# dohyeon-Lee/IsaacgymEnv

Hardware: AMD Instinct MI355X
Metric: env-steps/sec AnymalTerrain 4096 envs/GPU (higher is better)
Workload: dtype f32; 1 GPU; AnymalTerrain VecTask.step, terrainType plane (AnymalTerrain.yaml default), 5 physics substeps/step, obs noise on; num_envs_per_gpu=4096, global_num_envs=4096, parallelism=dp1, solver=TGS (physx.solver_type 1, cfg/config.yaml:31)

## Files before the change

isaacgymenv_amd/csrc/gs_capi.hip:

```cpp
#include <cmath>
#include <cstdio>
#include <cstring>
#include <algorithm>
#include <chrono>
#include <string>
#include <vector>

#include "gs_internal.h"
#include "../../include/gymsim.h"

namespace {
thread_local std::string g_err;

int fail(const char* fmt, const char* arg = nullptr) {
  char buf[512];
  std::snprintf(buf, sizeof(buf), fmt, arg ? arg : "");
  g_err = buf;
  return -1;
}
int hip_fail(hipError_t e, const char* where) {
  char buf[512];
  std::snprintf(buf, sizeof(buf), "%s: %s", where, hipGetErrorString(e));
  g_err = buf;
  return -1;
// ... 99 lines not shown
    if (hipError_t e = hipSetDevice(device); e != hipSuccess) {
      hip_fail(e, "gs_sim_create hipSetDevice");
      return nullptr;
    }
    s = new gs_sim();
    s->device = device;
  }
  s->params = *p;
  const int sub = p->substeps > 0 ? p->substeps : 1;
  s->dp.h = (float)(p->dt / sub);
  s->dp.substeps = sub;
  for (int k = 0; k < 3; ++k) s->dp.g[k] = (float)p->gravity[k];
  s->dp.pos_iters = p->num_position_iterations;
  s->dp.vel_iters = p->num_velocity_iterations;
  s->dp.contact_offset = (float)p->contact_offset;
  s->dp.rest_offset = (float)p->rest_offset;
  s->dp.max_depen_vel = (float)p->max_depenetration_velocity;
  s->dp.tgs = p->solver_type == 1 && p->num_position_iterations > 0 ? 1 : 0;
  s->dp.collect = p->contact_collection != 0;
  s->dp.limit_margin = (float)(p->joint_limit_margin > 0 ? p->joint_limit_margin : 0.0);
  s->dp.any_limits = 0;
  s->dp.has_ground = 0;
  s->dp.ground_mu = 1.f;
  return s;
}

void gs_sim_destroy(gs_sim* s) {
  if (!s) return;
  if (s->host) {
    host_pool_destroy(s->pool);
    delete s;
    return;
  }
  (void)hipSetDevice(s->device);
  if (s->d_model) (void)hipFree(s->d_model);
  if (s->d_links) (void)hipFree(s->d_links);
  if (s->d_tverts) (void)hipFree(s->d_tverts);
  if (s->d_tcells) (void)hipFree(s->d_tcells);
  if (s->d_tblk) (void)hipFree(s->d_tblk);
  if (s->d_tsq4) (void)hipFree(s->d_tsq4);
  if (s->d_trec) (void)hipFree(s->d_trec);
  if (s->d_rows) (void)hipFree(s->d_rows);
  if (s->d_gen) (void)hipFree(s->d_gen);
  if (s->ev0) (void)hipEventDestroy(s->ev0);
  if (s->ev1) (void)hipEventDestroy(s->ev1);
  delete s;
// ... 857 lines not shown
```

isaacgymenv_amd/csrc/gs_internal.h:

```cpp
#pragma once
#include <hip/hip_runtime.h>

#include "gs_terrain.h"
#include "../../include/gymtask.h"

#define GS_MAXB 32
#define GS_MAXD 32
#define GS_MAXC 192
#define GS_MAXL 40
#define GS_MAXS 8
#define GS_MAXSH 32
#define GS_MAXHV 2048
#define GS_MAXP 512
#define GS_MAXPV 512
#define GS_MAXPOOL 8
#define GS_WAVE 64
#ifndef GS_MIN_RESPONSE
#define GS_MIN_RESPONSE 1e-3f
#endif

struct DevModel {
  float jR[GS_MAXB][9];
  float jt[GS_MAXB][3];
  float jaxis[GS_MAXB][3];
// ... 29 lines not shown
struct DevParams {
  float h;
  int substeps;
  float g[3];
  int pos_iters, vel_iters;
  int tgs;
  float contact_offset, rest_offset, max_depen_vel;
  float ground_mu;
  int has_ground;
  int collect;
  float limit_margin;
  int any_limits;
  int has_terrain;
  TerrainDev terr;
  int any_drive;
  int self_collide;
  const float* ptgt;
  const float* vtgt;
  const float* dof_env;
  int dof_env_n;
  const struct GenTopo* gen;
  const struct DevLinks* gen_links;
  int gen_nd, gen_nr;
};
#define GS_DOFP_FIELDS 6

struct SimBuffers {
  float* state;
  const float* mu;
  float* cf;
  int N;
  float* sens;
  float* rows;
};

struct GenTopo {
  int nc;
  int cbody[GS_MAXC], cshape[GS_MAXC], clink[GS_MAXC];
};

struct PdDev {
  const float* actions;
  const float* dof_state_in;
  const float* default_pos;
  float kp, kd, scale, tlim;
  int decimation, extra;
// ... 103 lines not shown
```

isaacgymenv_amd/csrc/gs_team.hip:

```cpp
#include <type_traits>

#include "gs_internal.h"
#include "gs_topologies.h"
#include "gs_math.h"
#include "gs_pairs.h"
#include "gt_anymal_tail.h"

#ifdef GS_PHASE_PROFILE
__device__ unsigned long long gs_phase_cycles[64];
#define GS_PROF_DECL long long gs_t_ = clock64(); long long gs_acc_[16] = {0};
#define GS_PROF(i) { const long long t_ = clock64(); gs_acc_[i] += t_ - gs_t_; gs_t_ = t_; }
#define GS_PROF_COUNT(i, n) { gs_acc_[i] += (n); }
#define GS_PROF_PARAM , long long &gs_t_, long long *gs_acc_
#define GS_PROF_ARGS , gs_t_, gs_acc_
#define GS_PROF_FLUSH                                                   \
  if ((threadIdx.x & 63) == 0) {                                        \
    long long tot_ = 0;                                                 \
    for (int i_ = 0; i_ < 16; ++i_) {                                   \
      atomicAdd(&gs_phase_cycles[i_], (unsigned long long)gs_acc_[i_]); \
      if (i_ < 8 || i_ == 11) tot_ += gs_acc_[i_];                      \
    }                                                                   \
    atomicAdd(&gs_phase_cycles[16 + (int)min(tot_ / 25000, 15ll)], 1ull); \
    if (tot_ > 250000) {                                                \
      for (int i_ = 0; i_ < 16; ++i_) atomicAdd(&gs_phase_cycles[32 + i_], (unsigned long long)gs_acc_[i_]); \
// ... 67 lines not shown
    case 2: return qperm_i<0xAA>(x);
    default: return qperm_i<0xFF>(x);
  }
}

template <class T>
struct CM {
  static constexpr int CL = T::T_CL, CC = T::T_CC;
  static constexpr int BODY = 25;
  static constexpr int CAND = BODY * CL;
  static constexpr int DOF = CAND + 4 * CC;
  static constexpr int SHP = DOF + 3 * CL;
  static constexpr int NP = SHP + (T::NPK > 0 ? 8 * T::T_SPC : 0);
  static constexpr int LANES = T::T_LANES;
};

#ifndef GS_TEAM_BLOCK
#define GS_TEAM_BLOCK 64
#endif
constexpr int kTeamBlock = GS_TEAM_BLOCK;
static_assert(kTeamBlock % 4 == 0 && kTeamBlock <= GS_WAVE, "a workgroup holds whole teams within one wave");

constexpr int RW = kTeamBlock + 1;

template <class T>
struct RowSlots {
  static constexpr int CL = T::T_CL;
  static constexpr int ZROW = 16;
  static constexpr int RZROW = 16;
  static constexpr int CSLOT = 15;
  __device__ static constexpr int zslot(int comp) { return comp < 6 ? 4 * (comp >> 1) + (comp & 1) : 4 * (comp - 6) + 2; }
  __device__ static constexpr int zs(int rr, int s) { return rr < 2 ? 2 * s + rr : 2 * ZROW + s; }
  static constexpr int C_DI = 3 * ZROW, C_G = C_DI + 3, C_TP = C_G + 3, C_TV = C_TP + 1,
                       C_MU = C_TV + 1, C_ACT = C_MU + 1, C_SEP = C_ACT + 1, PER_CONTACT = C_SEP + 1;
  static constexpr int R_DI = 3 * RZROW, R_G = R_DI + 3, R_TP = R_G + 3, R_TV = R_TP + 1,
                       R_MU = R_TV + 1, R_SEP = R_MU + 1, PER_ROOT = R_SEP + 1;
  static constexpr int CHAIN = PER_CONTACT * T::T_CC;
  static constexpr int ROOT = PER_ROOT * (T::T_RC > 0 ? T::T_RC : 1);
  static constexpr int P_Z = kPoolLam + 3, P_DI = P_Z + 15, P_G = P_DI + 3, P_TP = P_G + 3, P_TV = P_TP + 1,
                       P_CA = P_TV + 1, P_CB = P_CA + 1, PER_POOL = P_CB + 1;
  static constexpr int POOL = CHAIN + ROOT;
  static constexpr int TOTAL = POOL + PER_POOL * T::NPK;
  __device__ static constexpr int chain(int j) { return j * PER_CONTACT; }
  __device__ static constexpr int root(int j) { return CHAIN + j * PER_ROOT; }
};

// ... 304 lines not shown
  return -1;
}
template <class T>
__device__ __forceinline__ unsigned long long team_pair_bit(int lc, int ra, int ja, int dl, int jb) {
  unsigned long long bit = 0ull;
#pragma unroll
  for (int c = 0; c < 4; ++c) {
    const int a = ja < 0 ? ra : T::T_RS + c * T::T_SPC + ja;
    const int b = T::T_RS + ((c + dl) & 3) * T::T_SPC + jb;
    const int q = team_pair_index<T>(a, b);
    bit = lc == c ? (q >= 0 ? 1ull << q : 0ull) : bit;
  }
  return bit;
}
__device__ __forceinline__ unsigned long long quad_or64(unsigned long long m) {
  int lo = (int)(unsigned)m, hi = (int)(unsigned)(m >> 32);
  lo |= qperm_i<0xB1>(lo);
  hi |= qperm_i<0xB1>(hi);
  lo |= qperm_i<0x4E>(lo);
  hi |= qperm_i<0x4E>(hi);
  return ((unsigned long long)(unsigned)hi << 32) | (unsigned)lo;
}

template <class T>
__device__ __forceinline__ int team_narrow_replicated(const DevModel* __restrict__ M, const DevParams& P,
                                                   const float* __restrict__ mu_g, int N, int e, int lc,
                                                   const float (&R0)[9], const float (&R)[T::T_CL][9],
                                                   const float (&X)[T::T_CL][3], unsigned long long near,
                                                   float* __restrict__ shw_tab, const float* __restrict__ sct,
                                                   float* __restrict__ pool) {
  constexpr int TPW = kTeamsPerBlock;
  const int team = threadIdx.x >> 2;
  float* tab = shw_tab + team;
  __syncthreads();
#pragma unroll
  for (int j = 0; j < T::T_SPC; ++j) {
    const int sh = T::T_RS + lc * T::T_SPC + j;
    const int k = T::sh_body[T::T_RS + j] - 1;
    const float* ps = sct + ShapeTab<T>::POSE + 15 * sh;
    float Rs[9], t[3], c[3];
    mat3mul(R[k], ps, Rs);
    mat3vec(R[k], ps + 9, t);
    mat3vec(R[k], ps + 12, c);
#pragma unroll
    for (int f = 0; f < 9; ++f) tab[(kShW * sh + f) * TPW] = Rs[f];
#pragma unroll
    for (int f = 0; f < 3; ++f) {
      tab[(kShW * sh + 9 + f) * TPW] = X[k][f] + t[f];
      tab[(kShW * sh + 12 + f) * TPW] = X[k][f] + c[f];
    }
  }
  if (lc == 0) {
#pragma unroll
    for (int sh = 0; sh < T::T_RS; ++sh) {
      const float* ps = sct + ShapeTab<T>::POSE + 15 * sh;
      float Rs[9], t[3], c[3];
      mat3mul(R0, ps, Rs);
      mat3vec(R0, ps + 9, t);
      mat3vec(R0, ps + 12, c);
#pragma unroll
      for (int f = 0; f < 9; ++f) tab[(kShW * sh + f) * TPW] = Rs[f];
#pragma unroll
      for (int f = 0; f < 3; ++f) {
        tab[(kShW * sh + 9 + f) * TPW] = t[f];
        tab[(kShW * sh + 12 + f) * TPW] = c[f];
      }
    }
  }
  __syncthreads();
  const unsigned long long tmask = quad_or64(near);
  int cnt = 0;
  if (tmask) cnt = self_contacts<T, TPW, RW, RowSlots<T>::PER_POOL>(M, P, mu_g, N, e, tab, pool, ShapeConstsTab{sct},
                                                                    tmask);
  return cnt;
}

template <class T>
__device__ __forceinline__ int team_self_contacts(const DevModel* __restrict__ M, const float* __restrict__ cm,
                                                  const DevParams& P, const float* __restrict__ mu_g, int N, int e,
                                                  int lc, const float (&R0)[9], const float (&R)[T::T_CL][9],
                                                  const float (&X)[T::T_CL][3], float* __restrict__ shw_tab,
                                                  const float* __restrict__ sct, float* __restrict__ pool) {
  constexpr int TPW = kTeamsPerBlock, LN = T::T_LANES, SPC = T::T_SPC, RSH = T::T_RS;
  using C = CM<T>;
  const float off = P.contact_offset * 1.001f + 1e-5f;
  float p0[SPC][3], p1[SPC][3], rad[SPC], hl[SPC];
#pragma unroll
  for (int j = 0; j < SPC; ++j) {
    const int k = T::sh_body[RSH + j] - 1;
    const float* sp = cm + (C::SHP + 8 * j) * LN;
    const float l0[3] = {sp[0], sp[LN], sp[2 * LN]}, l1[3] = {sp[3 * LN], sp[4 * LN], sp[5 * LN]};
    mat3vec(R[k], l0, p0[j]);
    mat3vec(R[k], l1, p1[j]);
#pragma unroll
    for (int f = 0; f < 3; ++f) { p0[j][f] += X[k][f]; p1[j][f] += X[k][f]; }
    rad[j] = sp[6 * LN];
    hl[j] = sp[7 * LN];
  }
  static_assert(T::NPAIR <= 64, "the team's near-pair mask is 64 bits");
  unsigned long long near = 0ull;
  auto test = [&](const float* a0, const float* a1, float ra, float ha, bool sa, int, const float* b0, const float* b1,
                  float rb, float hb, bool sb, int, unsigned long long bit) {
    const float rr = ra + rb + off;
    float dc = 0.f;
#pragma unroll
    for (int k = 0; k < 3; ++k) {
// ... 49 lines not shown
          q0[j][g] = dl == 1 ? qperm<0x39>(p0[j][g]) : qperm<0x4E>(p0[j][g]);
          q1[j][g] = dl == 1 ? qperm<0x39>(p1[j][g]) : qperm<0x4E>(p1[j][g]);
        }
      }
      if (dl == 1 || lcv < 2) {
        const int lo = (lcv + dl) & 3;
#pragma unroll
        for (int j = 0; j < SPC; ++j)
#pragma unroll
          for (int j2 = 0; j2 < SPC; ++j2)
            if (team_pair<T>(RSH + j, RSH + SPC + j2))
              f(p0[j], p1[j], rad[j], hl[j], T::shkind[RSH + j] == 1, RSH + lcv * SPC + j, q0[j2], q1[j2], rad[j2],
                hl[j2], T::shkind[RSH + j2] == 1, RSH + lo * SPC + j2, team_pair_bit<T>(lcv, 0, j, dl, j2));
      }
    }
  };
  visit(lc, test);
  if (__ballot(near != 0ull) == 0ull) return 0;
#ifdef GS_PHASE_PROFILE
  if ((threadIdx.x & 63) == 0) atomicAdd(&gs_phase_cycles[12], 1ull);
  const long long np_t0 = clock64();
#endif
  if constexpr (!team_closed_form<T>()) {
    return team_narrow_replicated<T>(M, P, mu_g, N, e, lc, R0, R, X, near, shw_tab, sct, pool);
  } else {
  constexpr int kLC = team_lc<T>(), kSt = kTeamSt;
  constexpr int kNone = 0x7fffffff;
  const int wl = threadIdx.x & 63;
  const int team = threadIdx.x >> 2;
  float* lslot = shw_tab + wl;
  float* tstg = shw_tab + kLC * kSt * 64 + team;
  static_assert(kLC * kSt * 64 + T::NPK * kSt * TPW <= shw_size<T>(), "contact staging fits the table");
  __syncthreads();
  const float coff = P.contact_offset;
  int cnt = 0;
  int key[kLC];
#pragma unroll
  for (int i = 0; i < kLC; ++i) key[i] = kNone;
  auto narrow = [&](const float* a0_, const float* a1_, float ra_, float, bool sa, int ia, const float* b0_,
                    const float* b1_, float rb_, float, bool sb, int ib, unsigned long long bit) {
    if (!(near & bit)) return;
    const int q = __builtin_ctzll(bit);
    const bool sw = ia > ib;
    float a0[3], a1[3], b0[3], b1[3];
#pragma unroll
    for (int k = 0; k < 3; ++k) {
      a0[k] = sw ? b0_[k] : a0_[k]; a1[k] = sw ? b1_[k] : a1_[k];
      b0[k] = sw ? a0_[k] : b0_[k]; b1[k] = sw ? a1_[k] : b1_[k];
    }
    const float ra = sw ? rb_ : ra_, rb = sw ? ra_ : rb_;
    const int sha = sw ? ib : ia, shb = sw ? ia : ib;
    float pa[2][3], pb[2][3];
    int nct = 1;
    if (!sa && !sb) {
#pragma unroll
      for (int k = 0; k < 3; ++k) { pa[0][k] = a0[k]; pb[0][k] = b0[k]; }
// ... 52 lines not shown
        if (!(l > 1e-9f)) { f[0] = 0.f; f[1] = 0.f; f[2] = 1.f; l = 1.f; }
#pragma unroll
        for (int k = 0; k < 3; ++k) nn[k] = f[k] / l;
        dist = 0.f;
      } else {
        const float idist = __builtin_amdgcn_rsqf(d2);
#pragma unroll
        for (int k = 0; k < 3; ++k) nn[k] *= idist;
      }
      const float sep = dist - ra - rb;
      if (!(sep < coff)) continue;
      const int kn = 2 * q + c;
      int slot = cnt < kLC ? cnt : -1;
      if (cnt >= kLC) {
        int m = 0, km = key[0];
#pragma unroll
        for (int i = 1; i < kLC; ++i) {
          m = key[i] > km ? i : m;
          km = key[i] > km ? key[i] : km;
        }
        slot = kn < km ? m : -1;
      }
      if (slot >= 0) {
        float* o = lslot + kSt * slot * 64;
#pragma unroll
        for (int k = 0; k < 3; ++k) {
          o[k * 64] = 0.5f * ((pa[c][k] - ra * nn[k]) + (pb[c][k] + rb * nn[k]));
          o[(3 + k) * 64] = nn[k];
        }
        o[6 * 64] = sep;
        o[7 * 64] = __int_as_float(sha);
        o[8 * 64] = __int_as_float(shb);
#pragma unroll
        for (int i = 0; i < kLC; ++i) key[i] = i == slot ? kn : key[i];
      }
      ++cnt;
    }
  };
  visit(opaque_index(lc), narrow);
#ifdef GS_PHASE_PROFILE
  if ((threadIdx.x & 63) == 0) atomicAdd(&gs_phase_cycles[14], (unsigned long long)(clock64() - np_t0));
#endif
  int cnt_team = 0;
  {
    int rk[kLC];
#pragma unroll
    for (int i = 0; i < kLC; ++i) rk[i] = 0;
    auto tally = [&](const int (&ks)[kLC]) {
#pragma unroll
      for (int j = 0; j < kLC; ++j)
#pragma unroll
        for (int i = 0; i < kLC; ++i) rk[i] += ks[j] < key[i];
    };
    tally(key);
    {
      int ks[kLC];
#pragma unroll
      for (int j = 0; j < kLC; ++j) ks[j] = qperm_i<0x39>(key[j]);
      tally(ks);
#pragma unroll
      for (int j = 0; j < kLC; ++j) ks[j] = qperm_i<0x4E>(key[j]);
      tally(ks);
#pragma unroll
      for (int j = 0; j < kLC; ++j) ks[j] = qperm_i<0x93>(key[j]);
      tally(ks);
    }
    cnt_team = cnt + qperm_i<0xB1>(cnt);
    cnt_team += qperm_i<0x4E>(cnt_team);
#pragma unroll
    for (int i = 0; i < kLC; ++i) {
      if (i < cnt && rk[i] < T::NPK) {
        const float* src = lslot + kSt * i * 64;
        float* dst = tstg + kSt * rk[i] * TPW;
#pragma unroll
        for (int f = 0; f < kSt; ++f) dst[f * TPW] = src[f * 64];
      }
    }
    __syncthreads();
    cnt_team = cnt_team < T::NPK ? cnt_team : T::NPK;
#pragma unroll
    for (int r = 0; r < T::NPK; ++r) {
      if (r < cnt_team) {
        const float* src = tstg + kSt * r * TPW;
        float* o = pool + RowSlots<T>::PER_POOL * r * RW;
#pragma unroll
        for (int k = 0; k < 3; ++k) {
          o[(kPoolX + k) * RW] = src[k * TPW];
          o[(kPoolN + k) * RW] = src[(3 + k) * TPW];
        }
        o[kPoolSep * RW] = src[6 * TPW];
        const int a = __float_as_int(src[7 * TPW]), b = __float_as_int(src[8 * TPW]);
        const float nn[3] = {src[3 * TPW], src[4 * TPW], src[5 * TPW]};
        float t1[3], t2[3];
        gs_terrain::tangents(nn, t1, t2);
#pragma unroll
        for (int k = 0; k < 3; ++k) {
          o[(kPoolT1 + k) * RW] = t1[k];
          o[(kPoolT2 + k) * RW] = t2[k];
        }
        o[kPoolMu * RW] = 0.5f * (mu_g[a * N + e] + mu_g[b * N + e]);
        const int bla = (int)sct[kShC * a + 3], blb = (int)sct[kShC * b + 3];
// ... 14 lines not shown
      atomicAdd(&gs_phase_cycles[10], (unsigned long long)__popcll(tm));
    }
  }
#endif
  return cnt_team;
  }
}

__device__ __forceinline__ float terrain_candidate(const DevParams& P, const float* p, const float* x, float r,
                                                   float* nrm, float& smu) {
  const float cw[3] = {p[0] + x[0], p[1] + x[1], p[2] + x[2]};
  float dist = P.has_ground ? cw[2] - r : 3.0e38f;
  nrm[0] = 0.f; nrm[1] = 0.f; nrm[2] = 1.f;
  smu = P.ground_mu;
  float st, nt[3];
  if (gs_terrain::sphere_contact(P.terr, cw, r, r + P.contact_offset, st, nt) && st < dist) {
    dist = st;
    nrm[0] = nt[0]; nrm[1] = nt[1]; nrm[2] = nt[2];
    smu = P.terr.mu;
  }
  return dist;
}

template <class T, bool TERR, bool TGS>
__device__ __forceinline__ void substep_team(const DevModel* __restrict__ Min, const float* __restrict__ mdl,
                                             const DevParams& P, TeamState<T>& s, const float* tau,
                                             const float* __restrict__ mu_t, int N, int e, int lc,
                                             float* __restrict__ rows_own, const float* __restrict__ rows_team,
                                             float* __restrict__ cf_soa, bool collect,
                                             float* __restrict__ cf_aos, float* __restrict__ shw_tab,
                                             const float* __restrict__ sct, float* __restrict__ stash GS_PROF_PARAM) {
  constexpr int CL = T::T_CL, CC = T::T_CC, RC = T::T_RC, NCH = T::T_NCH, LN = T::T_LANES;
  static_assert(NCH == LN && LN == 4, "lane teams are DPP quads with one chain per lane");
  using C = CM<T>;
  using RS = RowSlots<T>;
  uintptr_t mp = reinterpret_cast<uintptr_t>(Min);
  asm volatile("" : "+s"(mp));
  const DevModel* __restrict__ M = reinterpret_cast<const DevModel*>(mp);
  const float* cm = mdl + lc;
  const float h = P.h;

  float R0[9];
  {
    const float inv = rsqrtf(s.quat[0] * s.quat[0] + s.quat[1] * s.quat[1] + s.quat[2] * s.quat[2] +
                             s.quat[3] * s.quat[3]);
    const float qn[4] = {s.quat[0] * inv, s.quat[1] * inv, s.quat[2] * inv, s.quat[3] * inv};
    quat_to_mat(qn, R0);
// ... 81 lines not shown
      qr[CC] = M->cradius[lc];
    }
    constexpr int kQItem = 9;
    static_assert(T::NPK > 0 && kShW * T::NS >= kQItem * (CC * LN + RC), "query list fits the pose table");
    float* ql = shw_tab;
    const int wl = threadIdx.x & 63;
    const unsigned long long below = (1ull << wl) - 1ull;
    int slot[NQ];
    int cnt = 0;
#ifdef GS_PHASE_PROFILE
    const long long tq0 = clock64();
#endif
#pragma unroll
    for (int q = 0; q < NQ; ++q) {
      const bool need = qv[q] && gs_terrain::may_contact(P.terr, qc[q], qr[q], qr[q] + P.contact_offset);
      const unsigned long long bal = __ballot(need);
      slot[q] = need ? cnt + __popcll(bal & below) : -1;
      if (need) {
        float* it = ql + slot[q] * kQItem;
        it[0] = qc[q][0]; it[1] = qc[q][1]; it[2] = qc[q][2]; it[3] = qr[q];
      }
      cnt += __popcll(bal);
    }
    __syncthreads();
#ifdef GS_PHASE_PROFILE
    const long long tq1 = clock64();
#endif
    const unsigned long long live = __ballot(true);
    const int nlive = __popcll(live);
    for (int i = __popcll(live & below); i < cnt; i += nlive) {
      float* it = ql + i * kQItem;
      const float cw[3] = {it[0], it[1], it[2]};
      const float r = it[3];
      float st = 0.f, nt[3] = {0.f, 0.f, 1.f};
      const bool found = gs_terrain::sphere_contact_scan(P.terr, cw, r, r + P.contact_offset, st, nt);
      it[4] = found ? 1.f : 0.f;
      it[5] = st;
      it[6] = nt[0]; it[7] = nt[1]; it[8] = nt[2];
    }
    __syncthreads();
#ifdef GS_PHASE_PROFILE
    if ((threadIdx.x & 63) == 0) {
      const long long tq2 = clock64();
      atomicAdd(&gs_phase_cycles[50], (unsigned long long)(tq1 - tq0));
      atomicAdd(&gs_phase_cycles[51], (unsigned long long)(tq2 - tq1));
      atomicAdd(&gs_phase_cycles[52], (unsigned long long)cnt);
    }
#endif
    float rd = 3.0e38f, rn[3] = {0.f, 0.f, 1.f}, rm = P.ground_mu;
#pragma unroll
    for (int q = 0; q < NQ; ++q) {
      float dist = P.has_ground ? qc[q][2] - qr[q] : 3.0e38f;
      float nrm[3] = {0.f, 0.f, 1.f};
      float smu = P.ground_mu;
      if (slot[q] >= 0) {
        const float* it = ql + slot[q] * kQItem;
        if (it[4] != 0.f && it[5] < dist) {
          dist = it[5];
          nrm[0] = it[6]; nrm[1] = it[7]; nrm[2] = it[8];
          smu = P.terr.mu;
        }
      }
      if (q < CC) {
// ... 37 lines not shown
    if (T::jkind[1 + k] == 1) {
      float sn, cs;
      sincosf(qj, &sn, &cs);
      const float Cc = 1.f - cs;
      float Rq[9];
      Rq[0] = cs + ax[0] * ax[0] * Cc;         Rq[1] = ax[0] * ax[1] * Cc - ax[2] * sn; Rq[2] = ax[0] * ax[2] * Cc + ax[1] * sn;
      Rq[3] = ax[1] * ax[0] * Cc + ax[2] * sn; Rq[4] = cs + ax[1] * ax[1] * Cc;         Rq[5] = ax[1] * ax[2] * Cc - ax[0] * sn;
      Rq[6] = ax[2] * ax[0] * Cc - ax[1] * sn; Rq[7] = ax[2] * ax[1] * Cc + ax[0] * sn; Rq[8] = cs + ax[2] * ax[2] * Cc;
      mat3mul(RJ, Rq, R[k]);
      S[k][0] = aw[0]; S[k][1] = aw[1]; S[k][2] = aw[2];
      cross3(X[k], aw, &S[k][3]);
    } else {
#pragma unroll
      for (int f = 0; f < 9; ++f) R[k][f] = RJ[f];
      X[k][0] += aw[0] * qj; X[k][1] += aw[1] * qj; X[k][2] += aw[2] * qj;
      S[k][0] = S[k][1] = S[k][2] = 0.f;
      S[k][3] = aw[0]; S[k][4] = aw[1]; S[k][5] = aw[2];
    }
  }
  GS_PROF(0)
  int npc = 0;
  float* pool = rows_own + RS::POOL * RW;
  if constexpr (T::NPK > 0) {
    if (P.self_collide) npc = team_self_contacts<T>(M, cm, P, mu_t, kTeamsPerBlock, 0, lc, R0, R, X, shw_tab, sct, pool);
  }
  GS_PROF(11)
#pragma unroll
  for (int k = 0; k < CL; ++k) {
    const float* Vp = k == 0 ? nub : V[k - 1];
    const float* Ap = k == 0 ? A0 : A[k - 1];
    const float* bp = cm + (k * C::BODY) * LN;
    const float qd = s.qd[k];
    float c6[6];
#pragma unroll
    for (int f = 0; f < 6; ++f) V[k][f] = Vp[f] + S[k][f] * qd;
    crm(V[k], S[k], c6);
#pragma unroll
    for (int f = 0; f < 6; ++f) A[k][f] = Ap[f] + c6[f] * qd;
    float com[3], Il[6];
#pragma unroll
    for (int f = 0; f < 3; ++f) com[f] = bp[(16 + f) * LN];
#pragma unroll
    for (int f = 0; f < 6; ++f) Il[f] = bp[(19 + f) * LN];
    body_inertia(R[k], X[k], bp[15 * LN], com, Il, Ic[k]);
    {
      float ia[6], iv[6], x6[6];
      spi_mul(Ic[k], A[k], ia);
// ... 469 lines not shown
        c21 += zc3[2][k] * zc3[1][k];
      }
      g10 += quad_sum(c10);
      g20 += quad_sum(c20);
      g21 += quad_sum(c21);
      float di[3];
#pragma unroll
      for (int rr = 0; rr < 3; ++rr) {
        di[rr] = dd[rr] > GS_MIN_RESPONSE ? __builtin_amdgcn_rcpf(dd[rr]) : 0.f;
        o[(RS::P_DI + rr) * RW] = di[rr];
        o[(kPoolLam + rr) * RW] = 0.f;
      }
      o[(RS::P_G + 0) * RW] = g10 * di[1];
      o[(RS::P_G + 1) * RW] = g20 * di[2];
      o[(RS::P_G + 2) * RW] = g21 * di[2];
      const float sc = o[kPoolSep * RW];
      const float tgt = -sc * inv_h;
      o[RS::P_TP * RW] = (sc < 0.f ? fminf(tgt, P.max_depen_vel) : tgt) * di[0];
      o[RS::P_TV * RW] = (sc < 0.f ? 0.f : tgt) * di[0];
      o[RS::P_CA * RW] = (float)ca;
      o[RS::P_CB * RW] = (float)(cb == ca ? -1 : cb);
    }
  }
  __syncthreads();

  GS_PROF(3)
  auto stash_io = [&](bool save) {
    int q = 0;
    auto io = [&](float& v) {
      if (save) stash[q * kTeamBlock] = v; else v = stash[q * kTeamBlock];
      ++q;
    };
#pragma unroll
    for (int k = 0; k < 6; ++k) {
#pragma unroll
      for (int b = 0; b < k; ++b) io(Mbb[k][b]);
      io(sDb[k]);
      io(nufb[k]);
    }
#pragma unroll
    for (int k = 0; k < CL; ++k) {
#pragma unroll
      for (int b = 0; b < 6; ++b) io(Mcb[k][b]);
#pragma unroll
      for (int j = 0; j < k; ++j) io(Mcc[k][j]);
      io(sDc[k]);
      io(nufc[k]);
// ... 194 lines not shown
#pragma unroll
      for (int c = 0; c < NCH; ++c) aC[c] += wC[c];
    }
    if (it == P.pos_iters - 1) {
      if constexpr (tgs) {
        const float inv_n = 1.f / (float)P.pos_iters;
        float mC[NCH];
#pragma unroll
        for (int c = 0; c < NCH; ++c) mC[c] = aC[c] * inv_n;
        gather_w<T>(lc, aA * inv_n, aA2 * inv_n, mC, wbp, wcp);
      } else {
        gather_w<T>(lc, wA, wA2, wC, wbp, wcp);
      }
    }
  }
  float wb[6], wc[CL];
  gather_w<T>(lc, wA, wA2, wC, wb, wc);
  if (P.pos_iters <= 0) {
#pragma unroll
    for (int b = 0; b < 6; ++b) wbp[b] = wb[b];
#pragma unroll
    for (int k = 0; k < CL; ++k) wcp[k] = wc[k];
  }
  __syncthreads();
  stash_io(false);

  GS_PROF(4)
  float nunb[6], nupb[6], nunc[CL], nupc[CL];
#pragma unroll
  for (int k = 0; k < 6; ++k) {
    float v = wb[k] * sDb[k], vp = wbp[k] * sDb[k];
#pragma unroll
    for (int b = 0; b < k; ++b) { v -= Mbb[k][b] * nunb[b]; vp -= Mbb[k][b] * nupb[b]; }
    nunb[k] = v;
    nupb[k] = vp;
  }
#pragma unroll
  for (int k = 0; k < CL; ++k) {
    float v = wc[k] * sDc[k], vp = wcp[k] * sDc[k];
#pragma unroll
    for (int b = 0; b < 6; ++b) { v -= Mcb[k][b] * nunb[b]; vp -= Mcb[k][b] * nupb[b]; }
#pragma unroll
    for (int j = 0; j < k; ++j) { v -= Mcc[k][j] * nunc[j]; vp -= Mcc[k][j] * nupc[j]; }
    nunc[k] = v;
    nupc[k] = vp;
  }
#pragma unroll
// ... 113 lines not shown
        float* o = cf_aos + (size_t)e * T::NB * 3;
        o[0] = f0; o[1] = f1; o[2] = f2;
      }
    }
  }
  GS_PROF(5)
}

template <class T>
__device__ __forceinline__ void team_com_velocity(const DevModel* __restrict__ M, const TeamState<T>& s, float* v) {
  float R[9], c[3], wc[3];
  quat_to_mat(s.quat, R);
  mat3vec(R, M->root_com, c);
  cross3(s.w, c, wc);
  v[0] = s.vo[0] + wc[0]; v[1] = s.vo[1] + wc[1]; v[2] = s.vo[2] + wc[2];
}

__device__ __forceinline__ int xcd_block(int b, int G) {
  constexpr int kXcd = 8;
  const int per = G / kXcd, rem = G % kXcd, x = b % kXcd, q = b / kXcd;
  return x * per + (x < rem ? x : rem) + q;
}

template <class T, bool TERR, bool TGS>
__global__ __launch_bounds__(kTeamBlock, 1) void k_simulate_team(const DevModel* __restrict__ M, DevParams P,
                                                                 SimBuffers B, const float* __restrict__ tau_aos) {
  constexpr int LN = T::T_LANES, CL = T::T_CL, ND = T::ND;
  __shared__ float mdl[CM<T>::NP * LN];
  __shared__ float rows[RowSlots<T>::TOTAL * RW];
  __shared__ float shw_tab[shw_size<T>()];
  __shared__ float sct[ShapeTab<T>::SIZE];
  __shared__ float mu_tab[T::NS * kTeamsPerBlock];
  __shared__ float stash_tab[team_stash_size<T>() * kTeamBlock];
  stage_chain_model<T>(M, mdl);
  stage_shape_consts<T>(M, sct);
  const int lc = threadIdx.x & (LN - 1);
  const int e = (xcd_block(blockIdx.x, gridDim.x) * kTeamBlock + threadIdx.x) / LN;
  for (int sh = lc; sh < T::NS; sh += LN)
    mu_tab[sh * kTeamsPerBlock + (threadIdx.x >> 2)] = e < B.N ? B.mu[(size_t)sh * B.N + e] : 1.f;
  __syncthreads();
  if (e >= B.N) return;
  const float* mu_t = mu_tab + (threadIdx.x >> 2);
  const int N = B.N;
  TeamState<T> s;
  team_load<T>(B.state, N, e, lc, s);
  float tau[CL];
#pragma unroll
  for (int k = 0; k < CL; ++k) tau[k] = tau_aos ? tau_aos[(size_t)e * ND + lc * CL + k] : 0.f;
  float* own = rows + threadIdx.x;
  const float* team = rows + (threadIdx.x & ~(LN - 1));
  GS_PROF_DECL
  for (int sstep = 0; sstep < P.substeps; ++sstep) {
    const bool last = (sstep == P.substeps - 1) && P.collect;
    substep_team<T, TERR, TGS>(M, mdl, P, s, tau, mu_t, N, e, lc, own, team, B.cf, last, nullptr, shw_tab, sct, stash_tab + threadIdx.x GS_PROF_ARGS);
  }
  team_store<T>(B.state, N, opaque_index(e), opaque_index(lc), s);
  GS_PROF_FLUSH
}

template <class T, bool TERR, bool TGS>
__global__ __launch_bounds__(kTeamBlock, 1) void k_pd_step_team(const DevModel* __restrict__ M, DevParams P,
                                                                SimBuffers B, PdDev A) {
  constexpr int LN = T::T_LANES, CL = T::T_CL, ND = T::ND, NB = T::NB;
  __shared__ float mdl[CM<T>::NP * LN];
  __shared__ float rows[RowSlots<T>::TOTAL * RW];
  __shared__ float shw_tab[shw_size<T>()];
  __shared__ float sct[ShapeTab<T>::SIZE];
  __shared__ float mu_tab[T::NS * kTeamsPerBlock];
  __shared__ float stash_tab[team_stash_size<T>() * kTeamBlock];
  stage_chain_model<T>(M, mdl);
  stage_shape_consts<T>(M, sct);
  const int lc = threadIdx.x & (LN - 1);
  const int e = (xcd_block(blockIdx.x, gridDim.x) * kTeamBlock + threadIdx.x) / LN;
  for (int sh = lc; sh < T::NS; sh += LN)
    mu_tab[sh * kTeamsPerBlock + (threadIdx.x >> 2)] = e < B.N ? B.mu[(size_t)sh * B.N + e] : 1.f;
  __syncthreads();
  if (e >= B.N) return;
  const float* mu_t = mu_tab + (threadIdx.x >> 2);
  const int N = B.N;
  TeamState<T> s;
  team_load<T>(B.state, N, e, lc, s);
  float tau[CL];
  float* own = rows + threadIdx.x;
  const float* team = rows + (threadIdx.x & ~(LN - 1));
  const int sub = P.substeps;
  const int n_pd = A.decimation * sub;
  const int total = (A.decimation + A.extra) * sub;
  auto dof0 = [&]() { return (size_t)opaque_index(e) * ND + lc * CL; };
  GS_PROF_DECL
  for (int it = 0; it < total; ++it) {
    if (it < n_pd && (it % sub) == 0) {
      const bool first = it == 0;
      const size_t d0 = dof0();
#pragma unroll
      for (int k = 0; k < CL; ++k) {
        const float qj = first ? A.dof_state_in[(d0 + k) * 2 + 0] : s.q[k];
        const float qdj = first ? A.dof_state_in[(d0 + k) * 2 + 1] : s.qd[k];
        const float aj = A.actions[d0 + k];
        tau[k] = clampf(A.kp * (A.scale * aj + A.default_pos[lc * CL + k] - qj) - A.kd * qdj, -A.tlim, A.tlim);
      }
    }
    const bool last = ((it % sub) == sub - 1) && P.collect;
    GS_PROF(6)
    float* cf_aos = (it == total - 1) ? A.cf_out : nullptr;
    substep_team<T, TERR, TGS>(M, mdl, P, s, tau, mu_t, N, e, lc, own, team, B.cf, last, cf_aos, shw_tab, sct, stash_tab + threadIdx.x GS_PROF_ARGS);
    if (it == n_pd - 1 && A.dof_out) {
      const size_t d0 = dof0();
#pragma unroll
      for (int k = 0; k < CL; ++k) {
        A.dof_out[(d0 + k) * 2 + 0] = s.q[k];
        A.dof_out[(d0 + k) * 2 + 1] = s.qd[k];
      }
    }
  }
  team_store<T>(B.state, N, opaque_index(e), opaque_index(lc), s);
  const size_t d0 = dof0();
#pragma unroll
  for (int k = 0; k < CL; ++k) A.torques_out[d0 + k] = tau[k];
  if (A.actions_copy) {
#pragma unroll
    for (int k = 0; k < CL; ++k) A.actions_copy[d0 + k] = A.actions[d0 + k];
  }
  if (A.root_out && lc == 0) {
    float* o = A.root_out + (size_t)e * 13;
    o[0] = s.p[0]; o[1] = s.p[1]; o[2] = s.p[2];
    o[3] = s.quat[0]; o[4] = s.quat[1]; o[5] = s.quat[2]; o[6] = s.quat[3];
    float v[3];
    team_com_velocity<T>(M, s, v);
    o[7] = v[0]; o[8] = v[1]; o[9] = v[2];
    o[10] = s.w[0]; o[11] = s.w[1]; o[12] = s.w[2];
  }
  if constexpr (!TERR) if (kTeamsPerBlock == 16 && A.tail_on) {
    __syncthreads();
    const bool reset = lc == 0 && (ND == 12 ? gt_tail::post_a_env<true, false, (ND == 12 ? 12 : 0)>(
                                                  A.tail_p, A.tail_b, gt_anymal_hound{}, e)
                                            : gt_tail::post_a_env<true, false>(A.tail_p, A.tail_b, gt_anymal_hound{}, e));
    const unsigned long long m = __ballot(reset);
    unsigned m16 = 0;
#pragma unroll
    for (int i = 0; i < kTeamsPerBlock; ++i) m16 |= (unsigned)((m >> (LN * i)) & 1ull) << i;
    const int e0 = e - (int)(threadIdx.x / LN);
    const unsigned long long live = __ballot(true);
    if ((int)(threadIdx.x & 63) == __ffsll((long long)live) - 1) {
      uint16_t* slices = reinterpret_cast<uint16_t*>(A.tail_b.reset_masks);
      slices[e0 / kTeamsPerBlock] = (uint16_t)m16;
      if (e0 + kTeamsPerBlock >= N)
        for (int q = e0 / kTeamsPerBlock + 1; q % 4 != 0; ++q) slices[q] = 0;
      gt_tail::publish_count(A.tail_b, (unsigned)__popc(m16), gridDim.x);
    }
  }
  GS_PROF(7)
  GS_PROF_FLUSH
}

}

bool team_fused_tail_available() { return kTeamsPerBlock == 16; }

template <class T>
hipError_t launch_sim_team(const DevModel* M, const DevParams& P, const SimBuffers& B, const float* tau,
                           hipStream_t st) {
  if constexpr (T::HAS_TEAM) {
    static_assert(T::NR == T::NB, "the lane team reports contact forces per body (no kept fixed-joint links)");
    const long lanes = (long)B.N * T::T_LANES;
    const int blocks = (int)((lanes + kTeamBlock - 1) / kTeamBlock);
    if (P.has_terrain && P.tgs)
      hipLaunchKernelGGL((k_simulate_team<T, true, true>), dim3(blocks), dim3(kTeamBlock), 0, st, M, P, B, tau);
    else if (P.has_terrain)
      hipLaunchKernelGGL((k_simulate_team<T, true, false>), dim3(blocks), dim3(kTeamBlock), 0, st, M, P, B, tau);
    else if (P.tgs)
      hipLaunchKernelGGL((k_simulate_team<T, false, true>), dim3(blocks), dim3(kTeamBlock), 0, st, M, P, B, tau);
    else
      hipLaunchKernelGGL((k_simulate_team<T, false, false>), dim3(blocks), dim3(kTeamBlock), 0, st, M, P, B, tau);
    return hipGetLastError();
  } else {
    return hipErrorInvalidConfiguration;
  }
}
template <class T>
hipError_t launch_pd_team(const DevModel* M, const DevParams& P, const SimBuffers& B, const PdDev& A, hipStream_t st) {
  if constexpr (T::HAS_TEAM) {
    const long lanes = (long)B.N * T::T_LANES;
    const int blocks = (int)((lanes + kTeamBlock - 1) / kTeamBlock);
    if (P.has_terrain && P.tgs)
      hipLaunchKernelGGL((k_pd_step_team<T, true, true>), dim3(blocks), dim3(kTeamBlock), 0, st, M, P, B, A);
    else if (P.has_terrain)
      hipLaunchKernelGGL((k_pd_step_team<T, true, false>), dim3(blocks), dim3(kTeamBlock), 0, st, M, P, B, A);
    else if (P.tgs)
      hipLaunchKernelGGL((k_pd_step_team<T, false, true>), dim3(blocks), dim3(kTeamBlock), 0, st, M, P, B, A);
    else
      hipLaunchKernelGGL((k_pd_step_team<T, false, false>), dim3(blocks), dim3(kTeamBlock), 0, st, M, P, B, A);
    return hipGetLastError();
  } else {
    return hipErrorInvalidConfiguration;
  }
}

#define GS_TEAM_ENTRY(T, SIG) {SIG, T::HAS_TEAM ? &launch_sim_team<T> : nullptr, T::HAS_TEAM ? &launch_pd_team<T> : nullptr},
TeamEntry g_team_kernels[] = {GS_FOR_EACH_TOPOLOGY(GS_TEAM_ENTRY)};
const int g_num_team_kernels = sizeof(g_team_kernels) / sizeof(g_team_kernels[0]);

extern "C" int gs_debug_phase_cycles(unsigned long long* out, int n, int reset) {
#ifdef GS_PHASE_PROFILE
  if (!out || n <= 0 || n > 64) return -1;
  if (hipDeviceSynchronize() != hipSuccess) return -1;
  if (hipMemcpyFromSymbol(out, HIP_SYMBOL(gs_phase_cycles), sizeof(unsigned long long) * n) != hipSuccess) return -1;
  if (reset) {
    unsigned long long z[64] = {0};
    if (hipMemcpyToSymbol(HIP_SYMBOL(gs_phase_cycles), z, sizeof(z)) != hipSuccess) return -1;
  }
  return 0;
#else
  (void)out; (void)n; (void)reset;
  return -1;
// ... 3 lines not shown
```

Before: 31.53 million env-steps/s.

## Split team workgroups into multiple waves with fewer envs per wave on plane

```diff
diff --git a/isaacgymenv_amd/csrc/gs_capi.hip b/isaacgymenv_amd/csrc/gs_capi.hip
--- a/isaacgymenv_amd/csrc/gs_capi.hip
+++ b/isaacgymenv_amd/csrc/gs_capi.hip
@@ -1,4 +1,5 @@
 #include <cmath>
+#include <cstdlib>
 #include <cstdio>
 #include <cstring>
 #include <algorithm>
@@ -145,6 +146,10 @@
   s->dp.any_limits = 0;
   s->dp.has_ground = 0;
   s->dp.ground_mu = 1.f;
+  if (const char* v = std::getenv("GS_TEAM_ENVS_PER_WAVE")) {
+    const int w = std::atoi(v);
+    s->dp.team_epw = w == 16 || w == 8 || w == 4 ? w : 0;
+  }
   return s;
 }
 
diff --git a/isaacgymenv_amd/csrc/gs_internal.h b/isaacgymenv_amd/csrc/gs_internal.h
--- a/isaacgymenv_amd/csrc/gs_internal.h
+++ b/isaacgymenv_amd/csrc/gs_internal.h
@@ -75,6 +75,7 @@
   const struct GenTopo* gen;
   const struct DevLinks* gen_links;
   int gen_nd, gen_nr;
+  int team_epw;
 };
 #define GS_DOFP_FIELDS 6
 
diff --git a/isaacgymenv_amd/csrc/gs_team.hip b/isaacgymenv_amd/csrc/gs_team.hip
--- a/isaacgymenv_amd/csrc/gs_team.hip
+++ b/isaacgymenv_amd/csrc/gs_team.hip
@@ -113,6 +113,31 @@
 static_assert(kTeamBlock % 4 == 0 && kTeamBlock <= GS_WAVE, "a workgroup holds whole teams within one wave");
 
 constexpr int RW = kTeamBlock + 1;
+
+template <int EPW>
+struct WaveForm {
+  static_assert(EPW == 16 || EPW == 8 || EPW == 4, "envs per wave");
+  static constexpr bool kWhole = EPW * 4 >= kTeamBlock;
+  static constexpr int TEAMS = kWhole ? kTeamBlock / 4 : EPW;
+  static constexpr int LANES = 4 * TEAMS;
+  static constexpr int WAVES = kTeamBlock / LANES;
+  static constexpr int THREADS = kWhole ? kTeamBlock : GS_WAVE * WAVES;
+};
+template <int EPW>
+__device__ __forceinline__ int team_column() {
+  if constexpr (WaveForm<EPW>::kWhole) return threadIdx.x;
+  else return (threadIdx.x / GS_WAVE) * WaveForm<EPW>::LANES + (threadIdx.x & (GS_WAVE - 1));
+}
+template <int EPW>
+__device__ __forceinline__ void team_sync() {
+  if constexpr (WaveForm<EPW>::kWhole) {
+    __syncthreads();
+  } else {
+    __builtin_amdgcn_fence(__ATOMIC_RELEASE, "workgroup");
+    __builtin_amdgcn_wave_barrier();
+    __builtin_amdgcn_fence(__ATOMIC_ACQUIRE, "workgroup");
+  }
+}
 
 template <class T>
 struct RowSlots {
@@ -463,17 +488,17 @@
   return ((unsigned long long)(unsigned)hi << 32) | (unsigned)lo;
 }
 
-template <class T>
+template <class T, int EPW>
 __device__ __forceinline__ int team_narrow_replicated(const DevModel* __restrict__ M, const DevParams& P,
                                                    const float* __restrict__ mu_g, int N, int e, int lc,
                                                    const float (&R0)[9], const float (&R)[T::T_CL][9],
                                                    const float (&X)[T::T_CL][3], unsigned long long near,
                                                    float* __restrict__ shw_tab, const float* __restrict__ sct,
                                                    float* __restrict__ pool) {
-  constexpr int TPW = kTeamsPerBlock;
-  const int team = threadIdx.x >> 2;
+  constexpr int TPW = WaveForm<EPW>::TEAMS;
+  const int team = (threadIdx.x & (GS_WAVE - 1)) >> 2;
   float* tab = shw_tab + team;
-  __syncthreads();
+  team_sync<EPW>();
 #pragma unroll
   for (int j = 0; j < T::T_SPC; ++j) {
     const int sh = T::T_RS + lc * T::T_SPC + j;
@@ -508,7 +533,7 @@
       }
     }
   }
-  __syncthreads();
+  team_sync<EPW>();
   const unsigned long long tmask = quad_or64(near);
   int cnt = 0;
   if (tmask) cnt = self_contacts<T, TPW, RW, RowSlots<T>::PER_POOL>(M, P, mu_g, N, e, tab, pool, ShapeConstsTab{sct},
@@ -516,13 +541,14 @@
   return cnt;
 }
 
-template <class T>
+template <class T, int EPW>
 __device__ __forceinline__ int team_self_contacts(const DevModel* __restrict__ M, const float* __restrict__ cm,
                                                   const DevParams& P, const float* __restrict__ mu_g, int N, int e,
                                                   int lc, const float (&R0)[9], const float (&R)[T::T_CL][9],
                                                   const float (&X)[T::T_CL][3], float* __restrict__ shw_tab,
                                                   const float* __restrict__ sct, float* __restrict__ pool) {
-  constexpr int TPW = kTeamsPerBlock, LN = T::T_LANES, SPC = T::T_SPC, RSH = T::T_RS;
+  constexpr int TPW = WaveForm<EPW>::TEAMS, WL = WaveForm<EPW>::kWhole ? 64 : WaveForm<EPW>::LANES;
+  constexpr int LN = T::T_LANES, SPC = T::T_SPC, RSH = T::T_RS;
   using C = CM<T>;
   const float off = P.contact_offset * 1.001f + 1e-5f;
   float p0[SPC][3], p1[SPC][3], rad[SPC], hl[SPC];
@@ -618,16 +644,17 @@
   const long long np_t0 = clock64();
 #endif
   if constexpr (!team_closed_form<T>()) {
-    return team_narrow_replicated<T>(M, P, mu_g, N, e, lc, R0, R, X, near, shw_tab, sct, pool);
+    return team_narrow_replicated<T, EPW>(M, P, mu_g, N, e, lc, R0, R, X, near, shw_tab, sct, pool);
   } else {
   constexpr int kLC = team_lc<T>(), kSt = kTeamSt;
   constexpr int kNone = 0x7fffffff;
   const int wl = threadIdx.x & 63;
-  const int team = threadIdx.x >> 2;
+  const int team = wl >> 2;
   float* lslot = shw_tab + wl;
-  float* tstg = shw_tab + kLC * kSt * 64 + team;
-  static_assert(kLC * kSt * 64 + T::NPK * kSt * TPW <= shw_size<T>(), "contact staging fits the table");
-  __syncthreads();
+  float* tstg = shw_tab + kLC * kSt * WL + team;
+  static_assert(kLC * kSt * WL + T::NPK * kSt * TPW <= shw_size<T>() / WaveForm<EPW>::WAVES,
+                "contact staging fits the wave's slice of the table");
+  team_sync<EPW>();
   const float coff = P.contact_offset;
   int cnt = 0;
   int key[kLC];
@@ -726,15 +753,15 @@
         slot = kn < km ? m : -1;
       }
       if (slot >= 0) {
-        float* o = lslot + kSt * slot * 64;
+        float* o = lslot + kSt * slot * WL;
 #pragma unroll
         for (int k = 0; k < 3; ++k) {
-          o[k * 64] = 0.5f * ((pa[c][k] - ra * nn[k]) + (pb[c][k] + rb * nn[k]));
-          o[(3 + k) * 64] = nn[k];
-        }
-        o[6 * 64] = sep;
-        o[7 * 64] = __int_as_float(sha);
-        o[8 * 64] = __int_as_float(shb);
+          o[k * WL] = 0.5f * ((pa[c][k] - ra * nn[k]) + (pb[c][k] + rb * nn[k]));
+          o[(3 + k) * WL] = nn[k];
+        }
+        o[6 * WL] = sep;
+        o[7 * WL] = __int_as_float(sha);
+        o[8 * WL] = __int_as_float(shb);
 #pragma unroll
         for (int i = 0; i < kLC; ++i) key[i] = i == slot ? kn : key[i];
       }
@@ -774,13 +801,13 @@
 #pragma unroll
     for (int i = 0; i < kLC; ++i) {
       if (i < cnt && rk[i] < T::NPK) {
-        const float* src = lslot + kSt * i * 64;
+        const float* src = lslot + kSt * i * WL;
         float* dst = tstg + kSt * rk[i] * TPW;
 #pragma unroll
-        for (int f = 0; f < kSt; ++f) dst[f * TPW] = src[f * 64];
-      }
-    }
-    __syncthreads();
+        for (int f = 0; f < kSt; ++f) dst[f * TPW] = src[f * WL];
+      }
+    }
+    team_sync<EPW>();
     cnt_team = cnt_team < T::NPK ? cnt_team : T::NPK;
 #pragma unroll
     for (int r = 0; r < T::NPK; ++r) {
@@ -841,7 +868,7 @@
   return dist;
 }
 
-template <class T, bool TERR, bool TGS>
+template <class T, bool TERR, bool TGS, int EPW>
 __device__ __forceinline__ void substep_team(const DevModel* __restrict__ Min, const float* __restrict__ mdl,
                                              const DevParams& P, TeamState<T>& s, const float* tau,
                                              const float* __restrict__ mu_t, int N, int e, int lc,
@@ -969,7 +996,7 @@
       }
       cnt += __popcll(bal);
     }
-    __syncthreads();
+    team_sync<EPW>();
 #ifdef GS_PHASE_PROFILE
     const long long tq1 = clock64();
 #endif
@@ -985,7 +1012,7 @@
       it[5] = st;
       it[6] = nt[0]; it[7] = nt[1]; it[8] = nt[2];
     }
-    __syncthreads();
+    team_sync<EPW>();
 #ifdef GS_PHASE_PROFILE
     if ((threadIdx.x & 63) == 0) {
       const long long tq2 = clock64();
@@ -1069,7 +1096,7 @@
   int npc = 0;
   float* pool = rows_own + RS::POOL * RW;
   if constexpr (T::NPK > 0) {
-    if (P.self_collide) npc = team_self_contacts<T>(M, cm, P, mu_t, kTeamsPerBlock, 0, lc, R0, R, X, shw_tab, sct, pool);
+    if (P.self_collide) npc = team_self_contacts<T, EPW>(M, cm, P, mu_t, kTeamsPerBlock, 0, lc, R0, R, X, shw_tab, sct, pool);
   }
   GS_PROF(11)
 #pragma unroll
@@ -1585,7 +1612,7 @@
       o[RS::P_CB * RW] = (float)(cb == ca ? -1 : cb);
     }
   }
-  __syncthreads();
+  team_sync<EPW>();
 
   GS_PROF(3)
   auto stash_io = [&](bool save) {
@@ -1826,7 +1853,7 @@
 #pragma unroll
     for (int k = 0; k < CL; ++k) wcp[k] = wc[k];
   }
-  __syncthreads();
+  team_sync<EPW>();
   stash_io(false);
 
   GS_PROF(4)
@@ -1986,8 +2013,25 @@
   return x * per + (x < rem ? x : rem) + q;
 }
 
-template <class T, bool TERR, bool TGS>
-__global__ __launch_bounds__(kTeamBlock, 1) void k_simulate_team(const DevModel* __restrict__ M, DevParams P,
+struct TeamLane {
+  int wave, col, lc, e;
+  bool on;
+};
+template <class T, int EPW>
+__device__ __forceinline__ TeamLane team_lane(int N) {
+  constexpr int LN = T::T_LANES;
+  static_assert(WaveForm<EPW>::WAVES == 1 || shw_size<T>() % WaveForm<EPW>::WAVES == 0, "every wave its own slice");
+  TeamLane t;
+  t.wave = WaveForm<EPW>::kWhole ? 0 : (int)(threadIdx.x / GS_WAVE);
+  t.col = team_column<EPW>();
+  t.lc = threadIdx.x & (LN - 1);
+  t.on = WaveForm<EPW>::kWhole || (int)(threadIdx.x & (GS_WAVE - 1)) < WaveForm<EPW>::LANES;
+  t.e = t.on ? (xcd_block(blockIdx.x, gridDim.x) * kTeamBlock + t.col) / LN : N;
+  return t;
+}
+
+template <class T, bool TERR, bool TGS, int EPW>
+__global__ __launch_bounds__(WaveForm<EPW>::THREADS, 1) void k_simulate_team(const DevModel* __restrict__ M, DevParams P,
                                                                  SimBuffers B, const float* __restrict__ tau_aos) {
   constexpr int LN = T::T_LANES, CL = T::T_CL, ND = T::ND;
   __shared__ float mdl[CM<T>::NP * LN];
@@ -1998,32 +2042,34 @@
   __shared__ float stash_tab[team_stash_size<T>() * kTeamBlock];
   stage_chain_model<T>(M, mdl);
   stage_shape_consts<T>(M, sct);
-  const int lc = threadIdx.x & (LN - 1);
-  const int e = (xcd_block(blockIdx.x, gridDim.x) * kTeamBlock + threadIdx.x) / LN;
-  for (int sh = lc; sh < T::NS; sh += LN)
-    mu_tab[sh * kTeamsPerBlock + (threadIdx.x >> 2)] = e < B.N ? B.mu[(size_t)sh * B.N + e] : 1.f;
+  const TeamLane tl = team_lane<T, EPW>(B.N);
+  const int lc = tl.lc, e = tl.e, col = tl.col;
+  if (tl.on)
+    for (int sh = lc; sh < T::NS; sh += LN)
+      mu_tab[sh * kTeamsPerBlock + (col >> 2)] = e < B.N ? B.mu[(size_t)sh * B.N + e] : 1.f;
   __syncthreads();
   if (e >= B.N) return;
-  const float* mu_t = mu_tab + (threadIdx.x >> 2);
+  const float* mu_t = mu_tab + (col >> 2);
+  float* shw_wave = shw_tab + tl.wave * (shw_size<T>() / WaveForm<EPW>::WAVES);
   const int N = B.N;
   TeamState<T> s;
   team_load<T>(B.state, N, e, lc, s);
   float tau[CL];
 #pragma unroll
   for (int k = 0; k < CL; ++k) tau[k] = tau_aos ? tau_aos[(size_t)e * ND + lc * CL + k] : 0.f;
-  float* own = rows + threadIdx.x;
-  const float* team = rows + (threadIdx.x & ~(LN - 1));
+  float* own = rows + col;
+  const float* team = rows + (col & ~(LN - 1));
   GS_PROF_DECL
   for (int sstep = 0; sstep < P.substeps; ++sstep) {
     const bool last = (sstep == P.substeps - 1) && P.collect;
-    substep_team<T, TERR, TGS>(M, mdl, P, s, tau, mu_t, N, e, lc, own, team, B.cf, last, nullptr, shw_tab, sct, stash_tab + threadIdx.x GS_PROF_ARGS);
+    substep_team<T, TERR, TGS, EPW>(M, mdl, P, s, tau, mu_t, N, e, lc, own, team, B.cf, last, nullptr, shw_wave, sct, stash_tab + col GS_PROF_ARGS);
   }
   team_store<T>(B.state, N, opaque_index(e), opaque_index(lc), s);
   GS_PROF_FLUSH
 }
 
-template <class T, bool TERR, bool TGS>
-__global__ __launch_bounds__(kTeamBlock, 1) void k_pd_step_team(const DevModel* __restrict__ M, DevParams P,
+template <class T, bool TERR, bool TGS, int EPW>
+__global__ __launch_bounds__(WaveForm<EPW>::THREADS, 1) void k_pd_step_team(const DevModel* __restrict__ M, DevParams P,
                                                                 SimBuffers B, PdDev A) {
   constexpr int LN = T::T_LANES, CL = T::T_CL, ND = T::ND, NB = T::NB;
   __shared__ float mdl[CM<T>::NP * LN];
@@ -2034,19 +2080,21 @@
   __shared__ float stash_tab[team_stash_size<T>() * kTeamBlock];
   stage_chain_model<T>(M, mdl);
   stage_shape_consts<T>(M, sct);
-  const int lc = threadIdx.x & (LN - 1);
-  const int e = (xcd_block(blockIdx.x, gridDim.x) * kTeamBlock + threadIdx.x) / LN;
-  for (int sh = lc; sh < T::NS; sh += LN)
-    mu_tab[sh * kTeamsPerBlock + (threadIdx.x >> 2)] = e < B.N ? B.mu[(size_t)sh * B.N + e] : 1.f;
+  const TeamLane tl = team_lane<T, EPW>(B.N);
+  const int lc = tl.lc, e = tl.e, col = tl.col;
+  if (tl.on)
+    for (int sh = lc; sh < T::NS; sh += LN)
+      mu_tab[sh * kTeamsPerBlock + (col >> 2)] = e < B.N ? B.mu[(size_t)sh * B.N + e] : 1.f;
   __syncthreads();
   if (e >= B.N) return;
-  const float* mu_t = mu_tab + (threadIdx.x >> 2);
+  const float* mu_t = mu_tab + (col >> 2);
+  float* shw_wave = shw_tab + tl.wave * (shw_size<T>() / WaveForm<EPW>::WAVES);
   const int N = B.N;
   TeamState<T> s;
   team_load<T>(B.state, N, e, lc, s);
   float tau[CL];
-  float* own = rows + threadIdx.x;
-  const float* team = rows + (threadIdx.x & ~(LN - 1));
+  float* own = rows + col;
+  const float* team = rows + (col & ~(LN - 1));
   const int sub = P.substeps;
   const int n_pd = A.decimation * sub;
   const int total = (A.decimation + A.extra) * sub;
@@ -2067,7 +2115,7 @@
     const bool last = ((it % sub) == sub - 1) && P.collect;
     GS_PROF(6)
     float* cf_aos = (it == total - 1) ? A.cf_out : nullptr;
-    substep_team<T, TERR, TGS>(M, mdl, P, s, tau, mu_t, N, e, lc, own, team, B.cf, last, cf_aos, shw_tab, sct, stash_tab + threadIdx.x GS_PROF_ARGS);
+    substep_team<T, TERR, TGS, EPW>(M, mdl, P, s, tau, mu_t, N, e, lc, own, team, B.cf, last, cf_aos, shw_wave, sct, stash_tab + col GS_PROF_ARGS);
     if (it == n_pd - 1 && A.dof_out) {
       const size_t d0 = dof0();
 #pragma unroll
@@ -2094,7 +2142,7 @@
     o[7] = v[0]; o[8] = v[1]; o[9] = v[2];
     o[10] = s.w[0]; o[11] = s.w[1]; o[12] = s.w[2];
   }
-  if constexpr (!TERR) if (kTeamsPerBlock == 16 && A.tail_on) {
+  if constexpr (!TERR && EPW == 16) if (kTeamsPerBlock == 16 && A.tail_on) {
     __syncthreads();
     const bool reset = lc == 0 && (ND == 12 ? gt_tail::post_a_env<true, false, (ND == 12 ? 12 : 0)>(
                                                   A.tail_p, A.tail_b, gt_anymal_hound{}, e)
@@ -2121,6 +2169,29 @@
 
 bool team_fused_tail_available() { return kTeamsPerBlock == 16; }
 
+constexpr int kTeamEpwPlane = 4, kTeamEpwTerr = 16;
+static int team_epw(const DevParams& P, bool tail) {
+  if (kTeamBlock != GS_WAVE || tail) return 16;
+  const int w = P.team_epw > 0 ? P.team_epw : (P.has_terrain ? kTeamEpwTerr : kTeamEpwPlane);
+  return w == 8 || w == 4 ? w : 16;
+}
+#define GS_TEAM_LAUNCH_EPW(K, EPW, ...)                                                                      \
+  do {                                                                                                       \
+    const dim3 g_((unsigned)blocks), b_((unsigned)WaveForm<EPW>::THREADS);                                   \
+    if (P.has_terrain && P.tgs) hipLaunchKernelGGL((K<T, true, true, EPW>), g_, b_, 0, st, __VA_ARGS__);     \
+    else if (P.has_terrain) hipLaunchKernelGGL((K<T, true, false, EPW>), g_, b_, 0, st, __VA_ARGS__);        \
+    else if (P.tgs) hipLaunchKernelGGL((K<T, false, true, EPW>), g_, b_, 0, st, __VA_ARGS__);                \
+    else hipLaunchKernelGGL((K<T, false, false, EPW>), g_, b_, 0, st, __VA_ARGS__);                          \
+  } while (0)
+#define GS_TEAM_LAUNCH(K, epw, ...)                              \
+  do {                                                           \
+    if constexpr (kTeamBlock == GS_WAVE) {                       \
+      if ((epw) == 8) { GS_TEAM_LAUNCH_EPW(K, 8, __VA_ARGS__); break; }  \
+      if ((epw) == 4) { GS_TEAM_LAUNCH_EPW(K, 4, __VA_ARGS__); break; }  \
+    }                                                            \
+    GS_TEAM_LAUNCH_EPW(K, 16, __VA_ARGS__);                      \
+  } while (0)
+
 template <class T>
 hipError_t launch_sim_team(const DevModel* M, const DevParams& P, const SimBuffers& B, const float* tau,
                            hipStream_t st) {
@@ -2128,14 +2199,7 @@
     static_assert(T::NR == T::NB, "the lane team reports contact forces per body (no kept fixed-joint links)");
     const long lanes = (long)B.N * T::T_LANES;
     const int blocks = (int)((lanes + kTeamBlock - 1) / kTeamBlock);
-    if (P.has_terrain && P.tgs)
-      hipLaunchKernelGGL((k_simulate_team<T, true, true>), dim3(blocks), dim3(kTeamBlock), 0, st, M, P, B, tau);
-    else if (P.has_terrain)
-      hipLaunchKernelGGL((k_simulate_team<T, true, false>), dim3(blocks), dim3(kTeamBlock), 0, st, M, P, B, tau);
-    else if (P.tgs)
-      hipLaunchKernelGGL((k_simulate_team<T, false, true>), dim3(blocks), dim3(kTeamBlock), 0, st, M, P, B, tau);
-    else
-      hipLaunchKernelGGL((k_simulate_team<T, false, false>), dim3(blocks), dim3(kTeamBlock), 0, st, M, P, B, tau);
+    GS_TEAM_LAUNCH(k_simulate_team, team_epw(P, false), M, P, B, tau);
     return hipGetLastError();
   } else {
     return hipErrorInvalidConfiguration;
@@ -2146,14 +2210,7 @@
   if constexpr (T::HAS_TEAM) {
     const long lanes = (long)B.N * T::T_LANES;
     const int blocks = (int)((lanes + kTeamBlock - 1) / kTeamBlock);
-    if (P.has_terrain && P.tgs)
-      hipLaunchKernelGGL((k_pd_step_team<T, true, true>), dim3(blocks), dim3(kTeamBlock), 0, st, M, P, B, A);
-    else if (P.has_terrain)
-      hipLaunchKernelGGL((k_pd_step_team<T, true, false>), dim3(blocks), dim3(kTeamBlock), 0, st, M, P, B, A);
-    else if (P.tgs)
-      hipLaunchKernelGGL((k_pd_step_team<T, false, true>), dim3(blocks), dim3(kTeamBlock), 0, st, M, P, B, A);
-    else
-      hipLaunchKernelGGL((k_pd_step_team<T, false, false>), dim3(blocks), dim3(kTeamBlock), 0, st, M, P, B, A);
+    GS_TEAM_LAUNCH(k_pd_step_team, team_epw(P, A.tail_on != 0), M, P, B, A);
     return hipGetLastError();
   } else {
     return hipErrorInvalidConfiguration;
```

Result: faster. 32.45 million env-steps/s (median of 6 runs) (+2.9%).
